# bdaiinstitute/vlfm

Measured on AMD Instinct MI355X. Metric: env-steps/s (VLM+value-map update), 640x480 RGB-D, higher is better.
Workload: dtype f16 ViT-g (f32 accumulate) + f32 Q-Former (split-f16, 22-bit); f32 confidence + f64 value maps; 1 GPU; configs[1] step x resident envs: BLIP-2 ITC + ValueMap+ObstacleMap+sort_waypoints; envs_per_gpu=256, global_envs=256, map=1000x1000 @ 20 px/m, parallelism=env-sharded x1, tuned_gemms=True, vit_gemm=hip:fc1, attention=hip

## Files before the change

### include/vlfm_amd.h

```cpp
#ifndef VLFM_AMD_H
#define VLFM_AMD_H

#include <stddef.h>
#include <stdint.h>

#ifdef __cplusplus
extern "C" {
#endif

typedef enum {
    VLFM_OK = 0,
    VLFM_ERR_INVALID = -1,
    VLFM_ERR_OUTSIDE_MAP = -2,
    VLFM_ERR_INDEX = -3,
    VLFM_ERR_HIP = -4,
    VLFM_ERR_CAPACITY = -5
} vlfm_status;

enum { VLFM_FUSE_DEFAULT = 0, VLFM_FUSE_REPLACE = 1, VLFM_FUSE_EQUAL_WEIGHTING = 2 };

const char* vlfm_last_error(void);
int vlfm_abi_version(void);

int vlfm_profile_enable(int on);
// ... 127 lines not shown
                                int out_dtype, int patch_size, void* stream);

int vlfm_itc_head_batched(const float* d_proj, int batch, int n_query, int proj_dim,
                          const float* d_text, float* d_out, void* stream);

#define VLFM_ITC_MAX_PROMPTS 8
int vlfm_itc_head_multi(const float* d_proj, int batch, int n_query, int proj_dim, const float* d_text_table, int n_text,
                        const int32_t* d_text_index, int n_prompts, float* d_out, void* stream);

int vlfm_layernorm_bias_f16(const void* d_x, const float* d_channel_bias, const void* d_gamma, const void* d_beta,
                            void* d_y, int rows, int dim, float eps, void* stream);

int vlfm_vit_attention_f16(const void* d_qkv, void* d_out, int batch, int tokens, int heads, int head_dim, float scale,
                           void* stream);

int vlfm_gemm_f16_nt(const void* d_x, const void* d_w, const void* d_bias, void* d_c, int m, int n, int k, int epilogue,
                     void* stream);

int vlfm_gemm_f16_pair_f32_nt(const void* d_x, const void* d_w_pair, const void* d_bias_f32, void* d_out, int m, int n_out, int k,
                              void* stream);

int vlfm_qformer_cross_attention_f32(const void* d_q, const void* d_kv_blocks, void* d_out, int batch, int tokens, int queries,
                                     int heads, int k_block0, int v_block0, int m_total, float scale, void* stream);

int vlfm_gemm_f16_tile_order(int m, int n, int group_m, int* out, int capacity_pairs);
int vlfm_gemm_f16_work_items(int m, int n, int grid, int* out, int capacity_pairs);

int vlfm_split_f32_to_f16_pair(const float* d_src, void* d_hi, void* d_lo, long long count, int* d_overflow, void* stream);
int vlfm_gemm_f32_nt(const float* d_x, const float* d_w, const float* d_bias, const float* d_residual, float* d_c, int m, int n,
                     int k, int activation, int precision, const void* d_w_hi, const void* d_w_lo, int* d_overflow, void* stream);


int vlfm_layernorm_rows_f32(const float* d_x, const float* d_gamma, const float* d_beta, float* d_out, int batch, int height,
                            int width, int channels, int window, float eps, void* stream);
int vlfm_window_reverse_add_f32(float* d_x, const float* d_windows, int batch, int height, int width, int channels, int window,
                                void* stream);
int vlfm_dwconv3x3_nhwc_f32(const float* d_x, const float* d_w9c, const float* d_bias, float* d_out, int batch, int height, int width,
                            int channels, void* stream);
int vlfm_window_attention_f32(const float* d_qkv, const float* d_bias_t, float* d_out, long long windows, int tokens, int heads,
                              float scale, void* stream);
int vlfm_layernorm_rows_shifted_f32(const float* d_x, const float* d_gamma, const float* d_beta, float* d_out, int batch, int height,
                                    int width, int channels, int window, float eps, int shift, int pad_zero, void* stream);
int vlfm_window_reverse_add_shifted_f32(float* d_x, const float* d_windows, int batch, int height, int width, int channels, int window,
                                        int shift, void* stream);
int vlfm_window_attention_masked_f32(const float* d_qkv, const float* d_bias_t, const float* d_mask_t, int windows_per_image, float* d_out,
                                     long long windows, int tokens, int heads, float scale, void* stream);
// ... 183 lines not shown
```

### vlfm_amd/_lib.py

```python
from __future__ import annotations

import ctypes
import os
import subprocess
from typing import Optional

_HERE = os.path.dirname(os.path.abspath(__file__))
LIB_PATH = os.path.join(_HERE, "libvlfm_amd.so")
SOURCES = ["value_map.hip", "depth_ingest.hip", "depth_holes.hip", "obstacle_map.hip", "vlm_ops.hip", "vit_attention.hip", "qformer_attention.hip", "detect_ops.hip", "object_cloud.hip", "gemm_f16.hip", "gemm_f32.hip", "conv_nhwc.hip", "sam_ops.hip", "map_render.hip", "jpeg_codec.hip", "jpeg_entropy.hip", "jpeg_decode.hip", "world_render.hip", "host.cpp"]

VLFM_OK = 0
VLFM_ERR_INVALID = -1
VLFM_ERR_OUTSIDE_MAP = -2
VLFM_ERR_INDEX = -3
VLFM_ERR_HIP = -4
VLFM_ERR_CAPACITY = -5

FUSION_TYPES = {"default": 0, "replace": 1, "equal_weighting": 2}


class VmPose(ctypes.Structure):
    _fields_ = [("inv_affine", ctypes.c_double * 6), ("row0", ctypes.c_int32), ("col0", ctypes.c_int32),
                ("env", ctypes.c_int32), ("reserved", ctypes.c_int32)]

# ... 78 lines not shown
        L.vlfm_profile_enable.argtypes = [ci]
        L.vlfm_host_wait_mode.argtypes = [ci]
        L.vlfm_profile_read.argtypes = [ctypes.c_char_p, ctypes.POINTER(cd), ctypes.POINTER(ci)]
        L.vlfm_value_map_pose_params.argtypes = [vp, vp, vp, ci, ci, ci, ci, vp, ctypes.POINTER(ci)]
        L.vlfm_cone_template_host.argtypes = [cd, cd, ci, cd, vp, ci, vp, ci, ctypes.POINTER(ci)]
        L.vlfm_tan_table_host.argtypes = [cd, ci, vp]
        L.vlfm_disc_rows_host.argtypes = [ci, vp]
        L.vlfm_cone_template_build.argtypes = [vp, vp, ci, ci, vp, vp, vp]
        L.vlfm_depth_ingest_batched.argtypes = [vp, ci, ci, ci, vp, vp, vp, ci, ci, vp, vp, vp, vp, vp]
        L.vlfm_selftest_div_exact.argtypes = [vp, ci, cd, vp, vp]
        L.vlfm_hole_scratch_bytes.argtypes = [ci, ci, ci, ci, ci]
        L.vlfm_hole_scratch_bytes.restype = ctypes.c_size_t
        L.vlfm_fill_small_holes_batched.argtypes = [vp, vp, ci, ci, ci, cd, vp, ctypes.c_size_t, ci, ci, vp, vp, vp, vp,
                                                    ci, vp, vp]
        L.vlfm_depth_scatter_holes_batched.argtypes = [vp, ci, ci, ci, vp, vp, vp, vp, ci, ci, vp, vp, vp]
        L.vlfm_fill_small_holes_rig_batched.argtypes = [vp, vp, ci, ci, ci, cd, vp, ctypes.c_size_t, ci, ci, vp, vp, vp, vp,
                                                        ci, vp, vp, ci, vp]
        L.vlfm_depth_scatter_holes_rig_batched.argtypes = [vp, ci, ci, ci, vp, vp, vp, vp, ci, ci, vp, vp, vp, vp]
        L.vlfm_layernorm_bias_f16.argtypes = [vp, vp, vp, vp, vp, ci, ci, ctypes.c_float, vp]
        L.vlfm_vit_attention_f16.argtypes = [vp, vp, ci, ci, ci, ci, ctypes.c_float, vp]
        L.vlfm_gemm_f16_nt.argtypes = [vp, vp, vp, vp, ci, ci, ci, ci, vp]
        L.vlfm_gemm_f16_pair_f32_nt.argtypes = [vp, vp, vp, vp, ci, ci, ci, vp]
        L.vlfm_qformer_cross_attention_f32.argtypes = [vp, vp, vp, ci, ci, ci, ci, ci, ci, ci, ctypes.c_float, vp]
        L.vlfm_gemm_f32_nt.argtypes = [vp, vp, vp, vp, vp, ci, ci, ci, ci, ci, vp, vp, vp, vp]
        L.vlfm_split_f32_to_f16_pair.argtypes = [vp, vp, vp, ctypes.c_longlong, vp, vp]
        L.vlfm_layernorm_rows_f32.argtypes = [vp, vp, vp, vp, ci, ci, ci, ci, ci, ctypes.c_float, vp]
        L.vlfm_window_reverse_add_f32.argtypes = [vp, vp, ci, ci, ci, ci, ci, vp]
        L.vlfm_dwconv3x3_nhwc_f32.argtypes = [vp, vp, vp, vp, ci, ci, ci, ci, vp]
        L.vlfm_window_attention_f32.argtypes = [vp, vp, vp, ctypes.c_longlong, ci, ci, ctypes.c_float, vp]
        L.vlfm_layernorm_rows_shifted_f32.argtypes = [vp, vp, vp, vp, ci, ci, ci, ci, ci, ctypes.c_float, ci, ci, vp]
        L.vlfm_window_reverse_add_shifted_f32.argtypes = [vp, vp, ci, ci, ci, ci, ci, ci, vp]
        L.vlfm_window_attention_masked_f32.argtypes = [vp, vp, vp, ci, vp, ctypes.c_longlong, ci, ci, ctypes.c_float, vp]
        L.vlfm_maxpool2x2_nhwc_f16.argtypes = [vp, vp, ci, ci, ci, ci, vp]
        L.vlfm_conv_nhwc_tile.argtypes = [ci, ci, ci, ci, ctypes.POINTER(ci), ctypes.POINTER(ci)]
        L.vlfm_conv_nhwc_f16.argtypes = [vp, vp, vp, vp, vp, ci, ci, ci, ci, ci, ci, ci, ci, ci, ci, vp]
        L.vlfm_value_map_update_fused_batched.argtypes = [vp, ci, vp, vp, vp, ci, vp, vp, ci, vp, vp, ci, ci, ci, cd, cd,
                                                          ci, ci, vp, vp, vp, vp, vp]
        L.vlfm_value_map_update_rig_batched.argtypes = [vp, ci, vp, vp, vp, ci, ci, ci, vp, vp, vp, ci, ci, ci, ci, ci, vp, vp,
                                                        vp, vp]
        L.vlfm_value_map_sort_waypoints_batched.argtypes = [vp, ci, ci, vp, ci, ci, vp, ci, vp, vp]
        L.vlfm_resample_coeffs_host.argtypes = [ci, ci, vp, vp, ci, ctypes.POINTER(ci)]
        L.vlfm_resample_coeffs_filter_host.argtypes = [ci, ci, ci, vp, vp, ci, ctypes.POINTER(ci)]
        L.vlfm_preprocess_sam_batched.argtypes = [vp, ci, ci, ci, ci, ci, vp, vp, ci, vp, vp, ci, vp, vp, ci, vp, vp, vp]
        L.vlfm_preprocess_rgb_batched.argtypes = [vp, ci, ci, ci, ci, vp, vp, ci, vp, vp, ci, vp, vp, vp, vp, ci, ci, vp]
        L.vlfm_itc_head_batched.argtypes = [vp, ci, ci, ci, vp, vp, vp]
        L.vlfm_itc_head_multi.argtypes = [vp, ci, ci, ci, vp, ci, vp, ci, vp, vp]
# ... 104 lines not shown
```

### vlfm_amd/csrc/host.cpp

```cpp
#include <cmath>
#include <cstdint>
#include <cstring>
#include <mutex>
#include <string>

#include "../../include/vlfm_amd.h"
#include "status.h"

namespace vlfm {
static thread_local std::string g_last_error;
void set_last_error(const char* msg) { g_last_error = msg ? msg : ""; }
}

extern "C" const char* vlfm_last_error(void) { return vlfm::g_last_error.c_str(); }
extern "C" int vlfm_abi_version(void) { return 16; }

namespace {

const double kPi = 3.141592653589793238462643383279502884;

inline long round_half_even(double v) { return std::lrint(v); }

float sin_deg_table(int deg) {
    static float tab[451];
    static std::once_flag once;
    std::call_once(once, [] {
        for (int i = 0; i <= 450; i++) tab[i] = (float)(std::round(std::sin(i * kPi / 180.0) * 1e7) / 1e7);
    });
    return tab[deg];
}

}

extern "C" int vlfm_value_map_pose_params(const double* h_tf, const double* h_yaw, const int32_t* h_env, int n,
                                          int map_size, int pixels_per_meter, int template_size,
                                          vlfm_vm_pose* h_out, int* bad_index) {
    if (!h_tf || !h_out || n < 0 || map_size <= 0 || template_size <= 0)
        return vlfm::fail(VLFM_ERR_INVALID, "value_map_pose_params: bad argument");
// ... 255 lines not shown
```

### vlfm_amd/csrc/qformer_attention.hip

```cpp
#include <hip/hip_runtime.h>
#include <stdint.h>

#include "../../include/vlfm_amd.h"
#include "profile.h"
#include "status.h"

namespace vlfm {

typedef float qa_f32x16 __attribute__((ext_vector_type(16)));
typedef float qa_f32x4 __attribute__((ext_vector_type(4)));
using qa_lds_ptr = __attribute__((address_space(3))) unsigned char*;
using qa_gbl_ptr = const __attribute__((address_space(1))) unsigned char*;

constexpr int QA_ROWB = 256;
constexpr int QA_MERGE_REGS = 34;
constexpr int QA_MERGE = 3 * QA_MERGE_REGS * 64 * 4;
constexpr int QA_MAX_T = 257, QA_MAX_Q = 32;

struct QaArgs {
    const float* q;
    const float* kv;
    float* out;
    int B, T, Q, heads, k_block0, v_block0, M_total;
    int rows_pad;
    float scale_log2e;
};

struct QaKernel {
    const QaArgs& a;
    unsigned char* smem;
    qa_lds_ptr lds;
    int lane, wave, col, g, voff;

    __device__ QaKernel(const QaArgs& a_, unsigned char* smem_) : a(a_), smem(smem_), lds((qa_lds_ptr)smem_) {
        lane = threadIdx.x & 63;
        wave = __builtin_amdgcn_readfirstlane(threadIdx.x >> 6);
        col = lane & 31;
        g = lane >> 5;
        voff = a.rows_pad * QA_ROWB;
    }
    __device__ inline const unsigned char* block(int block0, int b, int h) const {
        return reinterpret_cast<const unsigned char*>(a.kv + ((size_t)(block0 + h) * (size_t)a.M_total + (size_t)b * (size_t)a.T) * 64);
    }
    __device__ inline void issue_k(const unsigned char* kg, int row0, int n_ins) const {
        const int r4 = lane >> 4, p = lane & 15;
        for (int ins = 0; ins < n_ins; ins++) {
            const int row = row0 + 4 * ins + r4, src_row = min(row, a.T - 1);
            const int dst = __builtin_amdgcn_readfirstlane((row0 + 4 * ins) * QA_ROWB);
            __builtin_amdgcn_global_load_lds((qa_gbl_ptr)(kg + (size_t)src_row * QA_ROWB + ((p ^ (row & 15)) << 4)), lds + dst, 16, 0, 0);
        }
    }
    __device__ inline void issue_v(const unsigned char* vg, int row0, int n_ins) const {
        const int r4 = lane >> 4, p = lane & 15;
        for (int ins = 0; ins < n_ins; ins++) {
            const int row = row0 + 4 * ins + r4, src_row = min(row, a.T - 1);
            const int dst = __builtin_amdgcn_readfirstlane(voff + (row0 + 4 * ins) * QA_ROWB);
            __builtin_amdgcn_global_load_lds((qa_gbl_ptr)(vg + (size_t)src_row * QA_ROWB + ((p ^ (((row >> 2) & 1) << 3)) << 4)),
                                             lds + dst, 16, 0, 0);
        }
    }
    __device__ inline void issue_rows(const unsigned char* kg, const unsigned char* vg, int row0, int n_ins) const {
        issue_k(kg, row0, n_ins);
        issue_v(vg, row0, n_ins);
    }
    __device__ inline void load_q(int b, int h, float (&qn)[32]) const {
        const float* src = a.q + ((size_t)b * a.Q + min(col, a.Q - 1)) * ((size_t)a.heads * 64) + (size_t)h * 64 + 32 * g;
#pragma unroll
        for (int c = 0; c < 8; c++) {
            const qa_f32x4 v = *reinterpret_cast<const qa_f32x4*>(src + 4 * c);
            qn[4 * c] = v[0]; qn[4 * c + 1] = v[1]; qn[4 * c + 2] = v[2]; qn[4 * c + 3] = v[3];
        }
    }
};

__device__ __forceinline__ void qa_item(int w, int heads, int& b, int& h) {
    const int xcd = w & 7, idx = w >> 3;
    b = (idx / heads) * 8 + xcd;
    h = idx % heads;
}

__global__ __launch_bounds__(256) void qformer_cross_attention_kernel(QaArgs a) {
    extern __shared__ __attribute__((aligned(16))) unsigned char smem[];
    QaKernel k(a, smem);
    const int lane = k.lane, wave = k.wave, col = k.col, g = k.g;
    const int n_full = a.T >> 5, n_left = a.T & 31, left_wave = n_full & 3, left_ins = (n_left + 3) >> 2;
    const int stride = gridDim.x;
    const int moff = 2 * k.voff;
    int w = blockIdx.x, b, h;
    qa_item(w, a.heads, b, h);
// ... 132 lines not shown
                }
            }
            if (col < a.Q) {
                const float inv = 1.0f / l;
                float* orow = a.out + ((size_t)b * a.Q + col) * ((size_t)a.heads * 64) + (size_t)h * 64 + 4 * g;
#pragma unroll
                for (int q4 = 0; q4 < 4; q4++) {
                    const qa_f32x4 s0 = {o0[4 * q4] * inv, o0[4 * q4 + 1] * inv, o0[4 * q4 + 2] * inv, o0[4 * q4 + 3] * inv};
                    const qa_f32x4 s1 = {o1[4 * q4] * inv, o1[4 * q4 + 1] * inv, o1[4 * q4 + 2] * inv, o1[4 * q4 + 3] * inv};
                    *reinterpret_cast<qa_f32x4*>(orow + 8 * q4) = s0;
                    *reinterpret_cast<qa_f32x4*>(orow + 32 + 8 * q4) = s1;
                }
            }
            __builtin_amdgcn_s_waitcnt(0xC07F);
        }
        asm volatile("" ::: "memory");
        __builtin_amdgcn_s_barrier();
        asm volatile("" ::: "memory");
        if (!more) break;
        w = nw; b = nb; h = nh;
    }
}

}

using namespace vlfm;

extern "C" int vlfm_qformer_cross_attention_f32(const void* d_q, const void* d_kv_blocks, void* d_out, int batch, int tokens,
                                                int queries, int heads, int k_block0, int v_block0, int m_total, float scale,
                                                void* stream) {
    if (batch == 0) return VLFM_OK;
    if (!d_q || !d_kv_blocks || !d_out || batch < 0 || tokens < 1 || tokens > QA_MAX_T || queries < 1 || queries > QA_MAX_Q || heads < 1 ||
        k_block0 < 0 || v_block0 < 0 || (long long)batch * tokens > (long long)m_total)
        return fail(VLFM_ERR_INVALID, "qformer_cross_attention_f32: head width 64, 1-32 queries, 1-257 tokens, batch * tokens <= m_total");
    if ((((uintptr_t)d_q | (uintptr_t)d_kv_blocks | (uintptr_t)d_out) & 15) != 0)
        return fail(VLFM_ERR_INVALID, "qformer_cross_attention_f32: pointers must be 16-byte aligned");
    QaArgs a;
    a.q = (const float*)d_q; a.kv = (const float*)d_kv_blocks; a.out = (float*)d_out;
    a.B = batch; a.T = tokens; a.Q = queries; a.heads = heads; a.k_block0 = k_block0; a.v_block0 = v_block0; a.M_total = m_total;
    a.rows_pad = (tokens + 3) & ~3;
    a.scale_log2e = scale * 1.4426950408889634f;
    const size_t lds = 2 * (size_t)a.rows_pad * QA_ROWB + QA_MERGE;
    const void* fn = reinterpret_cast<const void*>(qformer_cross_attention_kernel);
    static LdsOptIn opt;
    if (!opt.ensure(fn, lds)) return fail(VLFM_ERR_HIP, "qformer_cross_attention_f32: cannot opt in to the LDS size");
    const long long items = (long long)((batch + 7) / 8) * 8 * heads;
    const int n_cu = device_cu_count() & ~7;
    const dim3 grid((unsigned)(items < n_cu ? items : n_cu)), block(256);
    VLFM_TIMED("qformer_cross_attention_kernel", stream);
    VLFM_KLAUNCH(qformer_cross_attention_kernel, grid, block, lds, stream, a);
    return check_launch("qformer_cross_attention_kernel");
}
```

### vlfm_amd/csrc/vlm_ops.hip

```cpp
#include <hip/hip_fp16.h>
#include <hip/hip_bf16.h>
#include <hip/hip_runtime.h>
#include <stdint.h>

#include <cmath>
#include <cstdlib>
#include <vector>

#include "../../include/vlfm_amd.h"
#include "profile.h"
#include "status.h"

namespace vlfm {

constexpr int PRECISION_BITS = 32 - 8 - 2;

__device__ inline unsigned char clip8(int v) {
    v >>= PRECISION_BITS;
    return (unsigned char)(v < 0 ? 0 : v > 255 ? 255 : v);
}

__global__ __launch_bounds__(256) void resample_h_kernel(const unsigned char* __restrict__ src, int H, int W, int O,
                                                         const int* __restrict__ bounds, const int* __restrict__ kk,
                                                         int ksize, unsigned char* __restrict__ dst) {
// ... 267 lines not shown
                }
            }
        }
#pragma unroll
        for (int off = 32; off > 0; off >>= 1) sq += __shfl_xor(sq, off, 64);
        const float rstd = rsqrtf(sq * inv_d + eps);
#pragma unroll
        for (int i = 0; i < NV; i++) {
            const int v = lane + 64 * i;
            if (v < nvec) {
                Half8 o;
#pragma unroll
                for (int j = 0; j < 4; j++) {
                    const float2 g2 = __half22float2(gm[i].h[j]), b2 = __half22float2(bt[i].h[j]);
                    o.h[j] = __floats2half2_rn((val(cur, i, 2 * j) - mean) * rstd * g2.x + b2.x,
                                               (val(cur, i, 2 * j + 1) - mean) * rstd * g2.y + b2.y);
                }
                reinterpret_cast<Half8*>(y + (size_t)r * D)[v] = o;
            }
        }
#pragma unroll
        for (int i = 0; i < NV; i++) { cur[i] = nxt[i]; nxt[i] = nx2[i]; }
    }
}

__global__ __launch_bounds__(512) void itc_head_kernel(const float* __restrict__ proj, int NQ, int P,
                                                       const float* __restrict__ text, float* __restrict__ out) {
    __shared__ float cos_q[64];
    const int b = blockIdx.x, lane = threadIdx.x & 63, wave = threadIdx.x >> 6, n_waves = blockDim.x >> 6;
    const float* t = text + (size_t)b * P;
    for (int q = wave; q < NQ; q += n_waves) {
        const float* p = proj + ((size_t)b * NQ + q) * P;
        float n2 = 0.0f, dt = 0.0f;
        for (int j = lane; j < P; j += 64) {
            const float v = p[j];
            n2 = fmaf(v, v, n2);
            dt = fmaf(v, t[j], dt);
        }
        for (int off = 32; off > 0; off >>= 1) {
            n2 += __shfl_down(n2, off, 64);
            dt += __shfl_down(dt, off, 64);
        }
        if (lane == 0) cos_q[q] = dt / fmaxf(sqrtf(n2), 1e-12f);
    }
    __syncthreads();
    if (wave == 0) {
// ... 235 lines not shown
}

extern "C" int vlfm_layernorm_bias_f16(const void* d_x, const float* d_channel_bias, const void* d_gamma, const void* d_beta,
                                       void* d_y, int rows, int dim, float eps, void* stream) {
    if (rows == 0) return VLFM_OK;
    if (!d_x || !d_gamma || !d_beta || !d_y || rows < 0 || dim <= 0 || dim % 8 != 0 || dim > 64 * 8 * LN_MAXV)
        return fail(VLFM_ERR_INVALID, "layernorm_bias_f16: dim must be a multiple of 8 and <= 2048");
    const int nvec = dim / 8, nv = (nvec + 63) / 64;
    int rpw = rows / 8192;
    rpw = rpw < 1 ? 1 : rpw > LN_ROWS ? LN_ROWS : rpw;
    const int waves = (rows + rpw - 1) / rpw;
    const dim3 grid((waves + 3) / 4), block(256);
    const __half* x = (const __half*)d_x; const __half* g = (const __half*)d_gamma; const __half* b = (const __half*)d_beta;
    __half* y = (__half*)d_y;
    VLFM_TIMED("layernorm_bias_f16_kernel", stream);
    switch (nv) {
        case 1: VLFM_KLAUNCH(layernorm_bias_f16_kernel<1>, grid, block, 0, (hipStream_t)stream, x, d_channel_bias, g, b, y, rows, dim, eps, rpw); break;
        case 2: VLFM_KLAUNCH(layernorm_bias_f16_kernel<2>, grid, block, 0, (hipStream_t)stream, x, d_channel_bias, g, b, y, rows, dim, eps, rpw); break;
        case 3: VLFM_KLAUNCH(layernorm_bias_f16_kernel<3>, grid, block, 0, (hipStream_t)stream, x, d_channel_bias, g, b, y, rows, dim, eps, rpw); break;
        default: VLFM_KLAUNCH(layernorm_bias_f16_kernel<4>, grid, block, 0, (hipStream_t)stream, x, d_channel_bias, g, b, y, rows, dim, eps, rpw); break;
    }
    return check_launch("layernorm_bias_f16_kernel");
}
```

### vlfm_amd/vlm/blip2itm.py

```python
from __future__ import annotations

import hashlib
import math
import os
import re
from dataclasses import dataclass
from typing import Dict, List, Optional, Sequence, Tuple

import numpy as np
import torch
import torch.nn as nn
import torch.nn.functional as F


@dataclass
class Blip2ITCConfig:
    image_size: int = 224
    patch_size: int = 14
    v_hidden: int = 1408
    v_layers: int = 39
    v_heads: int = 16
    v_mlp: int = 6144
    v_ln_eps: float = 1e-6
    q_hidden: int = 768
# ... 173 lines not shown

class _BertAttention(nn.Module):
    def __init__(self, hidden: int, kv_hidden: int, heads: int, eps: float):
        super().__init__()
        self.heads = heads
        self.query = nn.Linear(hidden, hidden)
        self.key = nn.Linear(kv_hidden, hidden)
        self.value = nn.Linear(kv_hidden, hidden)
        self.dense = nn.Linear(hidden, hidden)
        self.LayerNorm = nn.LayerNorm(hidden, eps=eps)
        self._kv_split = None
        self._qkv_fused = None

    def _project_kv_f16(self, kv16: torch.Tensor) -> Tuple[torch.Tensor, torch.Tensor]:
        if self._kv_split is None or self._kv_split[0].device != kv16.device:
            w1, w2, w3 = _exact_split3(torch.cat([self.key.weight, self.value.weight]))
            bias = torch.cat([self.key.bias, self.value.bias]).detach().float()
            self._kv_split = (w1.t(), w2.t(), w3.t(), bias)
        o = _split_gemm(kv16.reshape(-1, kv16.shape[-1]), self._kv_split[:3], self._kv_split[3])
        o = o.view(*kv16.shape[:-1], -1)
        hid = self.key.out_features
        return o[..., :hid], o[..., hid:]

    def forward(self, x: torch.Tensor, kv: Optional[torch.Tensor] = None, mask: Optional[torch.Tensor] = None,
                kv_proj: Optional[Tuple[torch.Tensor, torch.Tensor]] = None, kv_blocks=None) -> torch.Tensor:
        b, n, d = x.shape
        h = self.heads
        if kv_blocks is not None:
            from . import ops

            blocks, tokens, k_block0, v_block0 = kv_blocks
            q = _qlinear(x, self.query.weight, self.query.bias).contiguous()
            a = ops.qformer_cross_attention(q, blocks, tokens, h, k_block0, v_block0, (d // h) ** -0.5)
            return self.LayerNorm(_qlinear(a, self.dense.weight, self.dense.bias, residual=x))
        if kv_proj is not None:
            q = _qlinear(x, self.query.weight, self.query.bias).view(b, n, h, d // h).transpose(1, 2)
            k = kv_proj[0].reshape(b, -1, h, d // h).transpose(1, 2)
            v = kv_proj[1].reshape(b, -1, h, d // h).transpose(1, 2)
        elif kv is None and x.is_cuda and not self.training:
            if self._qkv_fused is None or self._qkv_fused[0].device != x.device or self._qkv_fused[0].dtype != x.dtype:
                self._qkv_fused = (torch.cat([self.query.weight, self.key.weight, self.value.weight]).detach(),
                                   torch.cat([self.query.bias, self.key.bias, self.value.bias]).detach())
            qkv = _qlinear(x, *self._qkv_fused).view(b, n, 3, h, d // h).permute(2, 0, 3, 1, 4)
            q, k, v = qkv[0], qkv[1], qkv[2]
        else:
            q = self.query(x).view(b, n, h, d // h).transpose(1, 2)
            if kv is not None and kv.dtype == torch.float16 and kv.is_cuda and self.key.weight.dtype == torch.float32:
                k, v = self._project_kv_f16(kv)
                src_len = kv.shape[1]
            else:
                src = x if kv is None else kv.to(x.dtype)
                k, v, src_len = self.key(src), self.value(src), src.shape[1]
            k = k.reshape(b, src_len, h, d // h).transpose(1, 2)
            v = v.reshape(b, src_len, h, d // h).transpose(1, 2)
        a = F.scaled_dot_product_attention(q, k, v, attn_mask=mask)
        return self.LayerNorm(_qlinear(a.transpose(1, 2).reshape(b, n, d), self.dense.weight, self.dense.bias,
                                       residual=x))


class _BertFFN(nn.Module):
    def __init__(self, hidden: int, inter: int, eps: float):
        super().__init__()
        self.up = nn.Linear(hidden, inter)
        self.down = nn.Linear(inter, hidden)
        self.LayerNorm = nn.LayerNorm(hidden, eps=eps)

# ... 17 lines not shown
    def __init__(self, cfg: Blip2ITCConfig):
        super().__init__()
        c = self.cfg = cfg
        n_patches = (c.image_size // c.patch_size) ** 2
        self.class_embedding = nn.Parameter(torch.zeros(1, 1, c.v_hidden))
        self.position_embedding = nn.Parameter(torch.zeros(1, n_patches + 1, c.v_hidden))
        self.patch_embedding = nn.Conv2d(3, c.v_hidden, c.patch_size, c.patch_size)
        self.blocks = nn.ModuleList([_VitBlock(c) for _ in range(c.v_layers)])
        self.post_layernorm = nn.LayerNorm(c.v_hidden, eps=c.v_ln_eps)
        self.query_tokens = nn.Parameter(torch.zeros(1, c.num_query_tokens, c.q_hidden))
        self.word_embeddings = nn.Embedding(c.vocab_size, c.q_hidden)
        self.position_embeddings = nn.Embedding(c.max_position_embeddings, c.q_hidden)
        self.q_layernorm = nn.LayerNorm(c.q_hidden, eps=c.q_ln_eps)
        self.q_layers = nn.ModuleList([_QFormerLayer(c, i) for i in range(c.q_layers)])
        self.vision_projection = nn.Linear(c.q_hidden, c.proj_dim)
        self.text_projection = nn.Linear(c.q_hidden, c.proj_dim)
        self.deferred_bias = True
        self._deferred_c: Optional[torch.Tensor] = None
        self.split_kv = True
        self.split_kv_min_rows = 32 * 257
        self._kv_all = None
        self.fused_cross_kv = True
        self._kv_pair = None

    def init_random(self, seed: int = 0) -> "Blip2ITCModel":
        dev = self.query_tokens.device
        g = torch.Generator(device=dev).manual_seed(seed)
        with torch.no_grad():
            for p in self.parameters():
                if p.dim() > 1:
                    p.copy_(torch.randn(p.shape, generator=g, device=dev) * 0.02)
                else:
                    p.zero_()
            for m in self.modules():
                if isinstance(m, nn.LayerNorm):
                    m.weight.fill_(1.0)
        self.weights_changed()
        return self

    def weights_changed(self) -> None:
        self._deferred_c = None
        self._kv_all = None
        self._kv_pair = None
        for layer in self.q_layers:
            layer.attention._qkv_fused = None
            if layer.crossattention is not None:
                layer.crossattention._kv_split = None

    def vision_dtype(self) -> torch.dtype:
        return self.patch_embedding.weight.dtype

    def set_precision(self, vision_dtype: torch.dtype = torch.float16) -> "Blip2ITCModel":
        for m in (self.patch_embedding, self.blocks, self.post_layernorm):
            m.to(vision_dtype)
        self.class_embedding.data = self.class_embedding.data.to(vision_dtype)
        self.position_embedding.data = self.position_embedding.data.to(vision_dtype)
        self.weights_changed()
        return self

    def load_hf_state_dict(self, sd: Dict[str, torch.Tensor]) -> None:
        own = dict(self.named_parameters())

        def put(name: str, src: str) -> None:
            with torch.no_grad():
                own[name].copy_(sd[src].to(own[name].dtype).reshape(own[name].shape))

# ... 102 lines not shown
        put("text_projection.bias", take("text_proj.bias"))
        unfed = sorted(set(own) - fed)
        if unfed:
            raise KeyError(f"{len(unfed)} parameters of the graph were not fed, e.g. {unfed[:4]}")

        def unused_ok(k: str) -> bool:
            return (k.startswith(("Qformer.cls.", "itm_head.")) or k in ("temp", "Qformer.bert.embeddings.position_ids")
                    or k.startswith(f"visual_encoder.blocks.{c.v_layers}.")
                    or k.startswith(("visual_encoder.norm.", "visual_encoder.fc_norm.", "visual_encoder.head.")))

        left = sorted(k for k in src if k not in used and not unused_ok(k))
        if left:
            raise KeyError(f"{len(left)} tensors of the file have no place in the ITC graph, e.g. {left[:4]}")
        self.weights_changed()

    def vision_tokens(self, pixel_values: torch.Tensor) -> torch.Tensor:
        c = self.cfg
        if pixel_values.dim() == 4:
            b, g = pixel_values.shape[0], c.image_size // c.patch_size
            pixel_values = pixel_values.reshape(b, 3, g, c.patch_size, g, c.patch_size).permute(0, 2, 4, 1, 3, 5) \
                .reshape(b, g * g, 3 * c.patch_size * c.patch_size)
        w = self.patch_embedding.weight
        x = F.linear(pixel_values.to(w.dtype), w.view(w.shape[0], -1), self.patch_embedding.bias)
        x = torch.cat([self.class_embedding.expand(x.shape[0], -1, -1), x], dim=1) + self.position_embedding
        if self.deferred_bias and x.is_cuda and x.dtype == torch.float16 and c.v_hidden % 8 == 0 and c.v_hidden <= 2048:
            from . import ops

            c = self._deferred_constants()
            x = x.contiguous()
            for i, blk in enumerate(self.blocks):
                x = blk.forward_deferred(x, c[2 * i], c[2 * i + 1])
            return ops.layernorm_bias(x, c[2 * len(self.blocks)], self.post_layernorm.weight, self.post_layernorm.bias,
                                      self.post_layernorm.eps)
        for blk in self.blocks:
            x = blk(x)
        return self.post_layernorm(x)

    def _deferred_constants(self) -> torch.Tensor:
        if self._deferred_c is None or self._deferred_c.device != self.post_layernorm.weight.device:
            rows, run = [], torch.zeros(self.cfg.v_hidden, dtype=torch.float32, device=self.post_layernorm.weight.device)
            for blk in self.blocks:
                rows.append(run.clone())
                run = run + blk.projection.bias.detach().float()
                rows.append(run.clone())
                run = run + blk.fc2.bias.detach().float()
            rows.append(run.clone())
            self._deferred_c = torch.stack(rows).contiguous()
        return self._deferred_c

    def query_features(self, image_tokens: torch.Tensor) -> torch.Tensor:
        split_ok = (self.split_kv and image_tokens.dtype == torch.float16 and image_tokens.is_cuda
                    and image_tokens.shape[0] * image_tokens.shape[1] >= self.split_kv_min_rows)
        enc = image_tokens if split_ok else image_tokens.to(self.q_layernorm.weight.dtype)
        h = self.q_layernorm(self.query_tokens).expand(enc.shape[0], -1, -1)
        fused = split_ok and self._fused_cross_ok(enc)
        blocks = self._project_all_kv_blocks(enc) if fused else None
        proj = self._project_all_kv(enc) if split_ok and not fused else None
        hid, at = self.cfg.q_hidden, 0
        for layer in self.q_layers:
            h = layer.attention(h)
            if layer.crossattention is not None:
                if blocks is not None:
                    h = layer.crossattention(h, kv_blocks=(blocks, enc.shape[1], at // 64, (at + hid) // 64))
                    at += 2 * hid
                elif proj is not None:
                    h = layer.crossattention(h, kv_proj=(proj[..., at:at + hid], proj[..., at + hid:at + 2 * hid]))
                    at += 2 * hid
                else:
                    h = layer.crossattention(h, kv=enc)
            h = layer.ffn_query(h)
        return h

    def _fused_cross_ok(self, tokens16: torch.Tensor) -> bool:
        from . import ops

        c = self.cfg
        return (self.fused_cross_kv and KV_SPLIT_PIECES == 2 and not torch.is_grad_enabled()
                and self.q_layernorm.weight.dtype == torch.float32
                and c.q_hidden % c.q_heads == 0 and c.q_hidden // c.q_heads == ops.QFORMER_ATTENTION_HEAD
                and c.num_query_tokens <= ops.QFORMER_ATTENTION_MAX_QUERIES
                and 1 <= tokens16.shape[1] <= ops.QFORMER_ATTENTION_MAX_TOKENS and c.v_hidden % 64 == 0
                and tokens16.shape[0] * tokens16.shape[1] * c.v_hidden * 2 < (1 << 32))

    def _kv_all_pieces(self, device):
        if self._kv_all is None or self._kv_all[0].device != device:
            cross = [l.crossattention for l in self.q_layers if l.crossattention is not None]
            w = torch.cat([torch.cat([c.key.weight, c.value.weight]) for c in cross])
            bias = torch.cat([torch.cat([c.key.bias, c.value.bias]) for c in cross]).detach().float()
            w1, w2, w3 = _exact_split3(w)
            self._kv_all = (w1.t(), w2.t(), w3.t(), bias)
            self._kv_pair = None
        return self._kv_all

    def _project_all_kv_blocks(self, tokens16: torch.Tensor) -> torch.Tensor:
        from . import ops

        w1t, w2t, _, bias = self._kv_all_pieces(tokens16.device)
        if self._kv_pair is None:
            self._kv_pair = (ops.interleave_pair_weights(w1t.t(), w2t.t()), bias.contiguous())
        return ops.linear_pair_f32(tokens16.reshape(-1, tokens16.shape[-1]), *self._kv_pair)

    def _project_all_kv(self, tokens16: torch.Tensor) -> torch.Tensor:
        pieces = self._kv_all_pieces(tokens16.device)
        o = _split_gemm(tokens16.reshape(-1, tokens16.shape[-1]), pieces[:3], pieces[3])
        return o.view(*tokens16.shape[:-1], -1)
# ... 303 lines not shown
```

### vlfm_amd/vlm/ops.py

```python
from __future__ import annotations

import ctypes
from typing import Dict, Optional, Tuple

import numpy as np
import torch

from .. import _lib

CLIP_MEAN = (0.48145466, 0.4578275, 0.40821073)
CLIP_STD = (0.26862954, 0.26130258, 0.27577711)
_DTYPE_CODE = {torch.float32: 0, torch.float16: 1, torch.bfloat16: 2}
_coeff_cache: Dict[Tuple[str, int, int], Tuple[torch.Tensor, torch.Tensor, int]] = {}


def _stream() -> int:
    return torch._C._cuda_getCurrentRawStream(torch._C._cuda_getDevice())


def resample_coeffs(in_size: int, out_size: int, bilinear: bool = False) -> Tuple[np.ndarray, np.ndarray, int]:
    bounds = np.zeros((out_size, 2), np.int32)
    cap = out_size * (2 * int(np.ceil(2.0 * max(1.0, in_size / out_size))) + 1)
    kk = np.zeros(cap, np.int32)
    ks = ctypes.c_int(0)
# ... 258 lines not shown
    return torch.stack([w1.reshape(n // 64, 64, k), w2.reshape(n // 64, 64, k)], dim=1).reshape(2 * n, k).contiguous()


def linear_pair_f32(x: torch.Tensor, w_pair: torch.Tensor, bias: Optional[torch.Tensor] = None,
                    out: Optional[torch.Tensor] = None) -> torch.Tensor:
    assert x.is_cuda and x.dtype == torch.float16 and x.is_contiguous() and x.dim() == 2
    assert w_pair.dtype == torch.float16 and w_pair.is_contiguous() and w_pair.shape[1] == x.shape[1] and w_pair.shape[0] % 128 == 0
    M, K = x.shape
    N = w_pair.shape[0] // 2
    assert bias is None or (bias.dtype == torch.float32 and bias.is_contiguous() and bias.numel() == N)
    if out is None:
        out = torch.empty((N // 64, M, 64), dtype=torch.float32, device=x.device)
    else:
        assert out.dtype == torch.float32 and out.is_contiguous() and out.shape == (N // 64, M, 64) and out.device == x.device
    _lib.check(_lib.lib().vlfm_gemm_f16_pair_f32_nt(x.data_ptr(), w_pair.data_ptr(), bias.data_ptr() if bias is not None else None,
                                                    out.data_ptr(), M, N, K, _stream()), "gemm_f16_pair_f32_nt")
    return out


QFORMER_ATTENTION_MAX_TOKENS, QFORMER_ATTENTION_MAX_QUERIES, QFORMER_ATTENTION_HEAD = 257, 32, 64


def qformer_cross_attention(q: torch.Tensor, kv_blocks: torch.Tensor, tokens: int, heads: int, k_block0: int, v_block0: int,
                            scale: float, out: Optional[torch.Tensor] = None) -> torch.Tensor:
    assert q.is_cuda and q.dtype == torch.float32 and q.is_contiguous() and q.dim() == 3 and q.shape[2] == heads * 64
    assert kv_blocks.dtype == torch.float32 and kv_blocks.is_contiguous() and kv_blocks.dim() == 3 and kv_blocks.shape[2] == 64
    assert kv_blocks.device == q.device and max(k_block0, v_block0) + heads <= kv_blocks.shape[0] and min(k_block0, v_block0) >= 0
    B, Q, _ = q.shape
    if out is None:
        out = torch.empty_like(q)
    else:
        assert out.dtype == torch.float32 and out.is_contiguous() and out.shape[1:] == q.shape[1:] and out.shape[0] >= B
    _lib.check(_lib.lib().vlfm_qformer_cross_attention_f32(q.data_ptr(), kv_blocks.data_ptr(), out.data_ptr(), B, tokens, Q, heads,
                                                           k_block0, v_block0, kv_blocks.shape[1], float(scale), _stream()),
               "qformer_cross_attention_f32")
    return out


VIT_ATTENTION_TOKENS, VIT_ATTENTION_HEADS = 257, (88,)


def vit_attention(qkv: torch.Tensor, batch: int, tokens: int, heads: int, head_dim: int, scale: float) -> torch.Tensor:
    assert qkv.is_cuda and qkv.dtype == torch.float16 and qkv.is_contiguous()
    assert qkv.numel() == batch * tokens * 3 * heads * head_dim
    out = torch.empty((batch * tokens, heads * head_dim), dtype=torch.float16, device=qkv.device)
    _lib.check(_lib.lib().vlfm_vit_attention_f16(qkv.data_ptr(), out.data_ptr(), batch, tokens, heads, head_dim,
                                                 float(scale), _stream()), "vit_attention_f16")
    return out


_ACT32 = {None: 0, "none": 0, "relu": 1, "gelu": 2}
GEMM_F32_PRECISION = {"exact": 0, "split": 1}
_overflow_flags: Dict[tuple, torch.Tensor] = {}
_split_cache: Dict[int, tuple] = {}


def gemm_f32_overflow_flag(device, owner: str = "") -> torch.Tensor:
    d = torch.device(device)
# ... 114 lines not shown
```

Before: 1743 env-steps/s.

## Fold Q-Former layer-0 query prefix, add native self-attention and token-assembly kernels

The first Q-Former layer's self-attention and cross-attention query projection depend only on learned query tokens, so they are precomputed once and cached. A stride-0 Q path in the cross-attention kernel lets every image share the one cached query. A fused HIP kernel now handles Q-Former self-attention for the remaining layers, and a second kernel merges the ViT cls-token concat with the position-embedding add. Together these cut per-step GEMMs, launches and temporary tensors. The cost is cached state that must be invalidated when weights change.

```diff
diff --git a/include/vlfm_amd.h b/include/vlfm_amd.h
--- a/include/vlfm_amd.h
+++ b/include/vlfm_amd.h
@@ -173,6 +173,14 @@
 
 int vlfm_qformer_cross_attention_f32(const void* d_q, const void* d_kv_blocks, void* d_out, int batch, int tokens, int queries,
                                      int heads, int k_block0, int v_block0, int m_total, float scale, void* stream);
+int vlfm_qformer_cross_attention_strided_f32(const void* d_q, long long q_image_stride, const void* d_kv_blocks, void* d_out, int batch,
+                                             int tokens, int queries, int heads, int k_block0, int v_block0, int m_total, float scale,
+                                             void* stream);
+
+int vlfm_qformer_self_attention_f32(const void* d_qkv, void* d_out, int batch, int queries, int heads, float scale, void* stream);
+
+int vlfm_vit_assemble_tokens_f16(const void* d_patch, const void* d_cls, const void* d_pos, void* d_out, int batch, int patches,
+                                 int dim, void* stream);
 
 int vlfm_gemm_f16_tile_order(int m, int n, int group_m, int* out, int capacity_pairs);
 int vlfm_gemm_f16_work_items(int m, int n, int grid, int* out, int capacity_pairs);
diff --git a/vlfm_amd/_lib.py b/vlfm_amd/_lib.py
--- a/vlfm_amd/_lib.py
+++ b/vlfm_amd/_lib.py
@@ -124,6 +124,10 @@
         L.vlfm_gemm_f16_nt.argtypes = [vp, vp, vp, vp, ci, ci, ci, ci, vp]
         L.vlfm_gemm_f16_pair_f32_nt.argtypes = [vp, vp, vp, vp, ci, ci, ci, vp]
         L.vlfm_qformer_cross_attention_f32.argtypes = [vp, vp, vp, ci, ci, ci, ci, ci, ci, ci, ctypes.c_float, vp]
+        L.vlfm_qformer_cross_attention_strided_f32.argtypes = [vp, ctypes.c_longlong, vp, vp, ci, ci, ci, ci, ci, ci, ci,
+                                                               ctypes.c_float, vp]
+        L.vlfm_qformer_self_attention_f32.argtypes = [vp, vp, ci, ci, ci, ctypes.c_float, vp]
+        L.vlfm_vit_assemble_tokens_f16.argtypes = [vp, vp, vp, vp, ci, ci, ci, vp]
         L.vlfm_gemm_f32_nt.argtypes = [vp, vp, vp, vp, vp, ci, ci, ci, ci, ci, vp, vp, vp, vp]
         L.vlfm_split_f32_to_f16_pair.argtypes = [vp, vp, vp, ctypes.c_longlong, vp, vp]
         L.vlfm_layernorm_rows_f32.argtypes = [vp, vp, vp, vp, ci, ci, ci, ci, ci, ctypes.c_float, vp]
diff --git a/vlfm_amd/csrc/host.cpp b/vlfm_amd/csrc/host.cpp
--- a/vlfm_amd/csrc/host.cpp
+++ b/vlfm_amd/csrc/host.cpp
@@ -13,7 +13,7 @@
 }
 
 extern "C" const char* vlfm_last_error(void) { return vlfm::g_last_error.c_str(); }
-extern "C" int vlfm_abi_version(void) { return 16; }
+extern "C" int vlfm_abi_version(void) { return 17; }
 
 namespace {
 
diff --git a/vlfm_amd/csrc/qformer_attention.hip b/vlfm_amd/csrc/qformer_attention.hip
--- a/vlfm_amd/csrc/qformer_attention.hip
+++ b/vlfm_amd/csrc/qformer_attention.hip
@@ -23,6 +23,7 @@
     float* out;
     int B, T, Q, heads, k_block0, v_block0, M_total;
     int rows_pad;
+    long long q_stride;
     float scale_log2e;
 };
 
@@ -64,7 +65,7 @@
         issue_v(vg, row0, n_ins);
     }
     __device__ inline void load_q(int b, int h, float (&qn)[32]) const {
-        const float* src = a.q + ((size_t)b * a.Q + min(col, a.Q - 1)) * ((size_t)a.heads * 64) + (size_t)h * 64 + 32 * g;
+        const float* src = a.q + (size_t)b * (size_t)a.q_stride + (size_t)min(col, a.Q - 1) * ((size_t)a.heads * 64) + (size_t)h * 64 + 32 * g;
 #pragma unroll
         for (int c = 0; c < 8; c++) {
             const qa_f32x4 v = *reinterpret_cast<const qa_f32x4*>(src + 4 * c);
@@ -243,23 +244,99 @@
     }
 }
 
+constexpr int QS_MAX_Q = 32;
+constexpr int QS_ROW = 68, QS_PROW = 33;
+
+__global__ __launch_bounds__(256) void qformer_self_attention_kernel(const float* __restrict__ qkv, float* __restrict__ out, int NQ,
+                                                                     int heads, float scale_log2e) {
+    __shared__ __attribute__((aligned(16))) float ks[QS_MAX_Q * QS_ROW];
+    __shared__ __attribute__((aligned(16))) float vs[QS_MAX_Q * QS_ROW];
+    __shared__ float ps[QS_MAX_Q * QS_PROW];
+    const int t = threadIdx.x, b = blockIdx.x / heads, h = blockIdx.x % heads;
+    const size_t hidden = (size_t)heads * 64, ld = 3 * hidden;
+    const float* base = qkv + (size_t)b * NQ * ld + (size_t)h * 64;
+    for (int r = t >> 4; r < NQ; r += 16) {
+        const int c = (t & 15) * 4;
+        *reinterpret_cast<qa_f32x4*>(ks + r * QS_ROW + c) = *reinterpret_cast<const qa_f32x4*>(base + r * ld + hidden + c);
+        *reinterpret_cast<qa_f32x4*>(vs + r * QS_ROW + c) = *reinterpret_cast<const qa_f32x4*>(base + r * ld + 2 * hidden + c);
+    }
+    const int i = t >> 3, part = t & 7;
+    qa_f32x4 q[16];
+    {
+        const float* qrow = base + (size_t)min(i, NQ - 1) * ld;
+#pragma unroll
+        for (int c = 0; c < 16; c++) q[c] = *reinterpret_cast<const qa_f32x4*>(qrow + 4 * c);
+    }
+    __syncthreads();
+    float s[4], m = -INFINITY;
+#pragma unroll
+    for (int jj = 0; jj < 4; jj++) {
+        const int j = part + 8 * jj;
+        s[jj] = -INFINITY;
+        if (j < NQ) {
+            qa_f32x4 acc = {0.f, 0.f, 0.f, 0.f};
+#pragma unroll
+            for (int c = 0; c < 16; c++) {
+                const qa_f32x4 k4 = *reinterpret_cast<const qa_f32x4*>(ks + j * QS_ROW + 4 * c);
+#pragma unroll
+                for (int e = 0; e < 4; e++) acc[e] = fmaf(q[c][e], k4[e], acc[e]);
+            }
+            s[jj] = (acc[0] + acc[1]) + (acc[2] + acc[3]);
+        }
+        m = fmaxf(m, s[jj]);
+    }
+#pragma unroll
+    for (int off = 1; off < 8; off <<= 1) m = fmaxf(m, __shfl_xor(m, off, 64));
+    float l = 0.f;
+#pragma unroll
+    for (int jj = 0; jj < 4; jj++) {
+        const int j = part + 8 * jj;
+        if (j < NQ) {
+            const float p = __builtin_amdgcn_exp2f((s[jj] - m) * scale_log2e);
+            l += p;
+            ps[i * QS_PROW + j] = p;
+        }
+    }
+#pragma unroll
+    for (int off = 1; off < 8; off <<= 1) l += __shfl_xor(l, off, 64);
+    __syncthreads();
+    qa_f32x4 o0 = {0.f, 0.f, 0.f, 0.f}, o1 = {0.f, 0.f, 0.f, 0.f};
+    for (int j = 0; j < NQ; j++) {
+        const float p = ps[i * QS_PROW + j];
+        const qa_f32x4 v0 = *reinterpret_cast<const qa_f32x4*>(vs + j * QS_ROW + 8 * part);
+        const qa_f32x4 v1 = *reinterpret_cast<const qa_f32x4*>(vs + j * QS_ROW + 8 * part + 4);
+#pragma unroll
+        for (int e = 0; e < 4; e++) { o0[e] = fmaf(p, v0[e], o0[e]); o1[e] = fmaf(p, v1[e], o1[e]); }
+    }
+    if (i < NQ) {
+        const float inv = 1.0f / l;
+        float* orow = out + ((size_t)b * NQ + i) * hidden + (size_t)h * 64 + 8 * part;
+        const qa_f32x4 r0 = {o0[0] * inv, o0[1] * inv, o0[2] * inv, o0[3] * inv}, r1 = {o1[0] * inv, o1[1] * inv, o1[2] * inv, o1[3] * inv};
+        *reinterpret_cast<qa_f32x4*>(orow) = r0;
+        *reinterpret_cast<qa_f32x4*>(orow + 4) = r1;
+    }
+}
+
 }
 
 using namespace vlfm;
 
-extern "C" int vlfm_qformer_cross_attention_f32(const void* d_q, const void* d_kv_blocks, void* d_out, int batch, int tokens,
-                                                int queries, int heads, int k_block0, int v_block0, int m_total, float scale,
-                                                void* stream) {
+extern "C" int vlfm_qformer_cross_attention_strided_f32(const void* d_q, long long q_image_stride, const void* d_kv_blocks, void* d_out,
+                                                        int batch, int tokens, int queries, int heads, int k_block0, int v_block0,
+                                                        int m_total, float scale, void* stream) {
     if (batch == 0) return VLFM_OK;
     if (!d_q || !d_kv_blocks || !d_out || batch < 0 || tokens < 1 || tokens > QA_MAX_T || queries < 1 || queries > QA_MAX_Q || heads < 1 ||
         k_block0 < 0 || v_block0 < 0 || (long long)batch * tokens > (long long)m_total)
         return fail(VLFM_ERR_INVALID, "qformer_cross_attention_f32: head width 64, 1-32 queries, 1-257 tokens, batch * tokens <= m_total");
+    if (q_image_stride != 0 && (q_image_stride < (long long)queries * heads * 64 || (q_image_stride & 3) != 0))
+        return fail(VLFM_ERR_INVALID, "qformer_cross_attention_f32: q stride must be 0 or a multiple of 4 floats >= queries * heads * 64");
     if ((((uintptr_t)d_q | (uintptr_t)d_kv_blocks | (uintptr_t)d_out) & 15) != 0)
         return fail(VLFM_ERR_INVALID, "qformer_cross_attention_f32: pointers must be 16-byte aligned");
     QaArgs a;
     a.q = (const float*)d_q; a.kv = (const float*)d_kv_blocks; a.out = (float*)d_out;
     a.B = batch; a.T = tokens; a.Q = queries; a.heads = heads; a.k_block0 = k_block0; a.v_block0 = v_block0; a.M_total = m_total;
     a.rows_pad = (tokens + 3) & ~3;
+    a.q_stride = q_image_stride;
     a.scale_log2e = scale * 1.4426950408889634f;
     const size_t lds = 2 * (size_t)a.rows_pad * QA_ROWB + QA_MERGE;
     const void* fn = reinterpret_cast<const void*>(qformer_cross_attention_kernel);
@@ -272,3 +349,25 @@
     VLFM_KLAUNCH(qformer_cross_attention_kernel, grid, block, lds, stream, a);
     return check_launch("qformer_cross_attention_kernel");
 }
+
+extern "C" int vlfm_qformer_cross_attention_f32(const void* d_q, const void* d_kv_blocks, void* d_out, int batch, int tokens,
+                                                int queries, int heads, int k_block0, int v_block0, int m_total, float scale,
+                                                void* stream) {
+    return vlfm_qformer_cross_attention_strided_f32(d_q, (long long)queries * heads * 64, d_kv_blocks, d_out, batch, tokens, queries,
+                                                    heads, k_block0, v_block0, m_total, scale, stream);
+}
+
+extern "C" int vlfm_qformer_self_attention_f32(const void* d_qkv, void* d_out, int batch, int queries, int heads, float scale,
+                                               void* stream) {
+    if (batch == 0) return VLFM_OK;
+    if (!d_qkv || !d_out || batch < 0 || queries < 1 || queries > QS_MAX_Q || heads < 1 || heads > 1024 ||
+        (long long)batch * heads > 0x7fffffffLL)
+        return fail(VLFM_ERR_INVALID, "qformer_self_attention_f32: head width 64, 1-32 queries, batch * heads < 2^31");
+    if ((((uintptr_t)d_qkv | (uintptr_t)d_out) & 15) != 0)
+        return fail(VLFM_ERR_INVALID, "qformer_self_attention_f32: pointers must be 16-byte aligned");
+    const dim3 grid((unsigned)(batch * heads)), block(256);
+    VLFM_TIMED("qformer_self_attention_kernel", stream);
+    VLFM_KLAUNCH(qformer_self_attention_kernel, grid, block, 0, stream, (const float*)d_qkv, (float*)d_out, queries, heads,
+                 scale * 1.4426950408889634f);
+    return check_launch("qformer_self_attention_kernel");
+}
diff --git a/vlfm_amd/csrc/vlm_ops.hip b/vlfm_amd/csrc/vlm_ops.hip
--- a/vlfm_amd/csrc/vlm_ops.hip
+++ b/vlfm_amd/csrc/vlm_ops.hip
@@ -313,6 +313,26 @@
 #pragma unroll
         for (int i = 0; i < NV; i++) { cur[i] = nxt[i]; nxt[i] = nx2[i]; }
     }
+}
+
+__global__ __launch_bounds__(256) void vit_assemble_tokens_f16_kernel(const Half8* __restrict__ patch, const Half8* __restrict__ cls,
+                                                                      const Half8* __restrict__ pos, Half8* __restrict__ out, int P,
+                                                                      int nvec, long long total) {
+    const long long idx = (long long)blockIdx.x * 256 + threadIdx.x;
+    if (idx >= total) return;
+    const int v = (int)(idx % nvec);
+    const long long row = idx / nvec;
+    const int t = (int)(row % (P + 1));
+    const long long b = row / (P + 1);
+    const Half8 x = t == 0 ? cls[v] : patch[(b * P + (t - 1)) * nvec + v];
+    const Half8 e = pos[(long long)t * nvec + v];
+    Half8 o;
+#pragma unroll
+    for (int j = 0; j < 4; j++) {
+        const float2 xf = __half22float2(x.h[j]), ef = __half22float2(e.h[j]);
+        o.h[j] = __floats2half2_rn(xf.x + ef.x, xf.y + ef.y);
+    }
+    out[idx] = o;
 }
 
 __global__ __launch_bounds__(512) void itc_head_kernel(const float* __restrict__ proj, int NQ, int P,
@@ -594,3 +614,19 @@
     }
     return check_launch("layernorm_bias_f16_kernel");
 }
+
+extern "C" int vlfm_vit_assemble_tokens_f16(const void* d_patch, const void* d_cls, const void* d_pos, void* d_out, int batch,
+                                            int patches, int dim, void* stream) {
+    if (batch == 0) return VLFM_OK;
+    if (!d_patch || !d_cls || !d_pos || !d_out || batch < 0 || patches < 1 || dim <= 0 || dim % 8 != 0)
+        return fail(VLFM_ERR_INVALID, "vit_assemble_tokens_f16: dim must be a multiple of 8, patches >= 1");
+    if ((((uintptr_t)d_patch | (uintptr_t)d_cls | (uintptr_t)d_pos | (uintptr_t)d_out) & 15) != 0)
+        return fail(VLFM_ERR_INVALID, "vit_assemble_tokens_f16: pointers must be 16-byte aligned");
+    const int nvec = dim / 8;
+    const long long total = (long long)batch * (patches + 1) * nvec, blocks = (total + 255) / 256;
+    if (blocks > 0x7fffffffLL) return fail(VLFM_ERR_INVALID, "vit_assemble_tokens_f16: more than 2^31 workgroups");
+    VLFM_TIMED("vit_assemble_tokens_f16_kernel", stream);
+    VLFM_KLAUNCH(vit_assemble_tokens_f16_kernel, dim3((unsigned)blocks), dim3(256), 0, (hipStream_t)stream, (const Half8*)d_patch,
+                 (const Half8*)d_cls, (const Half8*)d_pos, (Half8*)d_out, patches, nvec, total);
+    return check_launch("vit_assemble_tokens_f16_kernel");
+}
diff --git a/vlfm_amd/vlm/blip2itm.py b/vlfm_amd/vlm/blip2itm.py
--- a/vlfm_amd/vlm/blip2itm.py
+++ b/vlfm_amd/vlm/blip2itm.py
@@ -219,16 +219,29 @@
         hid = self.key.out_features
         return o[..., :hid], o[..., hid:]
 
+    def native_self_ok(self, x: torch.Tensor) -> bool:
+        from . import ops
+
+        n, d = x.shape[-2], x.shape[-1]
+        return (x.is_cuda and x.dtype == torch.float32 and self.query.weight.dtype == torch.float32
+                and not torch.is_grad_enabled() and d % self.heads == 0 and d // self.heads == ops.QFORMER_ATTENTION_HEAD
+                and 1 <= n <= ops.QFORMER_ATTENTION_MAX_QUERIES)
+
     def forward(self, x: torch.Tensor, kv: Optional[torch.Tensor] = None, mask: Optional[torch.Tensor] = None,
-                kv_proj: Optional[Tuple[torch.Tensor, torch.Tensor]] = None, kv_blocks=None) -> torch.Tensor:
+                kv_proj: Optional[Tuple[torch.Tensor, torch.Tensor]] = None, kv_blocks=None,
+                q_shared: Optional[torch.Tensor] = None) -> torch.Tensor:
         b, n, d = x.shape
         h = self.heads
         if kv_blocks is not None:
             from . import ops
 
             blocks, tokens, k_block0, v_block0 = kv_blocks
-            q = _qlinear(x, self.query.weight, self.query.bias).contiguous()
-            a = ops.qformer_cross_attention(q, blocks, tokens, h, k_block0, v_block0, (d // h) ** -0.5)
+            if q_shared is not None:
+                a = ops.qformer_cross_attention(q_shared, blocks, tokens, h, k_block0, v_block0, (d // h) ** -0.5, batch=b)
+            else:
+                q = _qlinear(x, self.query.weight, self.query.bias)
+                a = ops.qformer_cross_attention(q if q.is_contiguous() else q.contiguous(), blocks, tokens, h, k_block0, v_block0,
+                                                (d // h) ** -0.5)
             return self.LayerNorm(_qlinear(a, self.dense.weight, self.dense.bias, residual=x))
         if kv_proj is not None:
             q = _qlinear(x, self.query.weight, self.query.bias).view(b, n, h, d // h).transpose(1, 2)
@@ -238,7 +251,13 @@
             if self._qkv_fused is None or self._qkv_fused[0].device != x.device or self._qkv_fused[0].dtype != x.dtype:
                 self._qkv_fused = (torch.cat([self.query.weight, self.key.weight, self.value.weight]).detach(),
                                    torch.cat([self.query.bias, self.key.bias, self.value.bias]).detach())
-            qkv = _qlinear(x, *self._qkv_fused).view(b, n, 3, h, d // h).permute(2, 0, 3, 1, 4)
+            qkv = _qlinear(x, *self._qkv_fused)
+            if mask is None and self.native_self_ok(x) and qkv.is_contiguous():
+                from . import ops
+
+                a = ops.qformer_self_attention(qkv.view(b * n, 3 * d), b, n, h, (d // h) ** -0.5)
+                return self.LayerNorm(_qlinear(a.view(b, n, d), self.dense.weight, self.dense.bias, residual=x))
+            qkv = qkv.view(b, n, 3, h, d // h).permute(2, 0, 3, 1, 4)
             q, k, v = qkv[0], qkv[1], qkv[2]
         else:
             q = self.query(x).view(b, n, h, d // h).transpose(1, 2)
@@ -302,6 +321,9 @@
         self._kv_all = None
         self.fused_cross_kv = True
         self._kv_pair = None
+        self.fold_query_prefix = True
+        self._prefix = None
+        self._prefix_residual = {}
 
     def init_random(self, seed: int = 0) -> "Blip2ITCModel":
         dev = self.query_tokens.device
@@ -322,6 +344,8 @@
         self._deferred_c = None
         self._kv_all = None
         self._kv_pair = None
+        self._prefix = None
+        self._prefix_residual = {}
         for layer in self.q_layers:
             layer.attention._qkv_fused = None
             if layer.crossattention is not None:
@@ -470,12 +494,18 @@
                 .reshape(b, g * g, 3 * c.patch_size * c.patch_size)
         w = self.patch_embedding.weight
         x = F.linear(pixel_values.to(w.dtype), w.view(w.shape[0], -1), self.patch_embedding.bias)
-        x = torch.cat([self.class_embedding.expand(x.shape[0], -1, -1), x], dim=1) + self.position_embedding
+        if (x.is_cuda and x.dtype == torch.float16 and c.v_hidden % 8 == 0 and not torch.is_grad_enabled() and x.is_contiguous()
+                and self.class_embedding.dtype == self.position_embedding.dtype == torch.float16):
+            from . import ops
+
+            x = ops.vit_assemble_tokens(x.view(-1, c.v_hidden), self.class_embedding.view(-1),
+                                        self.position_embedding.view(-1, c.v_hidden), x.shape[0])
+        else:
+            x = (torch.cat([self.class_embedding.expand(x.shape[0], -1, -1), x], dim=1) + self.position_embedding).contiguous()
         if self.deferred_bias and x.is_cuda and x.dtype == torch.float16 and c.v_hidden % 8 == 0 and c.v_hidden <= 2048:
             from . import ops
 
             c = self._deferred_constants()
-            x = x.contiguous()
             for i, blk in enumerate(self.blocks):
                 x = blk.forward_deferred(x, c[2 * i], c[2 * i + 1])
             return ops.layernorm_bias(x, c[2 * len(self.blocks)], self.post_layernorm.weight, self.post_layernorm.bias,
@@ -505,7 +535,15 @@
         blocks = self._project_all_kv_blocks(enc) if fused else None
         proj = self._project_all_kv(enc) if split_ok and not fused else None
         hid, at = self.cfg.q_hidden, 0
-        for layer in self.q_layers:
+        fold = fused and self._fold_prefix_ok(enc.shape[0])
+        for i, layer in enumerate(self.q_layers):
+            if i == 0 and fold:
+                _, q0 = self._query_prefix(enc.device)
+                h = layer.crossattention(self._prefix_rows(enc.shape[0], enc.device), q_shared=q0,
+                                         kv_blocks=(blocks, enc.shape[1], at // 64, (at + hid) // 64))
+                at += 2 * hid
+                h = layer.ffn_query(h)
+                continue
             h = layer.attention(h)
             if layer.crossattention is not None:
                 if blocks is not None:
@@ -529,6 +567,32 @@
                 and c.num_query_tokens <= ops.QFORMER_ATTENTION_MAX_QUERIES
                 and 1 <= tokens16.shape[1] <= ops.QFORMER_ATTENTION_MAX_TOKENS and c.v_hidden % 64 == 0
                 and tokens16.shape[0] * tokens16.shape[1] * c.v_hidden * 2 < (1 << 32))
+
+    def _fold_prefix_ok(self, batch: int) -> bool:
+        c, layer = self.cfg, self.q_layers[0]
+        if not (self.fold_query_prefix and layer.crossattention is not None and not torch.is_grad_enabled()):
+            return False
+        return (batch * c.num_query_tokens >= QFORMER_SPLIT_MIN_ROWS >= 64 and c.q_hidden % 32 == 0
+                and layer.attention.native_self_ok(self.query_tokens.detach()))
+
+    def _query_prefix(self, device) -> Tuple[torch.Tensor, torch.Tensor]:
+        if self._prefix is None or self._prefix[0].device != device:
+            n = self.cfg.num_query_tokens
+            copies = (QFORMER_SPLIT_MIN_ROWS + n - 1) // n
+            layer = self.q_layers[0]
+            with torch.no_grad():
+                s = layer.attention(self.q_layernorm(self.query_tokens).expand(copies, -1, -1))
+                q = _qlinear(s, layer.crossattention.query.weight, layer.crossattention.query.bias)
+                self._prefix = (s[0].clone(), q[0].clone())
+            self._prefix_residual = {}
+        return self._prefix
+
+    def _prefix_rows(self, batch: int, device) -> torch.Tensor:
+        s0, _ = self._query_prefix(device)
+        rows = self._prefix_residual.get(batch)
+        if rows is None or rows.device != s0.device:
+            rows = self._prefix_residual[batch] = s0.expand(batch, -1, -1).contiguous()
+        return rows
 
     def _kv_all_pieces(self, device):
         if self._kv_all is None or self._kv_all[0].device != device:
diff --git a/vlfm_amd/vlm/ops.py b/vlfm_amd/vlm/ops.py
--- a/vlfm_amd/vlm/ops.py
+++ b/vlfm_amd/vlm/ops.py
@@ -304,18 +304,44 @@
 
 
 def qformer_cross_attention(q: torch.Tensor, kv_blocks: torch.Tensor, tokens: int, heads: int, k_block0: int, v_block0: int,
-                            scale: float, out: Optional[torch.Tensor] = None) -> torch.Tensor:
-    assert q.is_cuda and q.dtype == torch.float32 and q.is_contiguous() and q.dim() == 3 and q.shape[2] == heads * 64
+                            scale: float, out: Optional[torch.Tensor] = None, batch: Optional[int] = None) -> torch.Tensor:
+    assert q.is_cuda and q.dtype == torch.float32 and q.is_contiguous() and q.shape[-1] == heads * 64
     assert kv_blocks.dtype == torch.float32 and kv_blocks.is_contiguous() and kv_blocks.dim() == 3 and kv_blocks.shape[2] == 64
     assert kv_blocks.device == q.device and max(k_block0, v_block0) + heads <= kv_blocks.shape[0] and min(k_block0, v_block0) >= 0
-    B, Q, _ = q.shape
+    if q.dim() == 2:
+        assert batch is not None and batch >= 0
+        B, Q, stride = int(batch), q.shape[0], 0
+    else:
+        assert q.dim() == 3 and (batch is None or batch == q.shape[0])
+        B, Q, stride = q.shape[0], q.shape[1], q.shape[1] * q.shape[2]
     if out is None:
-        out = torch.empty_like(q)
-    else:
-        assert out.dtype == torch.float32 and out.is_contiguous() and out.shape[1:] == q.shape[1:] and out.shape[0] >= B
-    _lib.check(_lib.lib().vlfm_qformer_cross_attention_f32(q.data_ptr(), kv_blocks.data_ptr(), out.data_ptr(), B, tokens, Q, heads,
-                                                           k_block0, v_block0, kv_blocks.shape[1], float(scale), _stream()),
-               "qformer_cross_attention_f32")
+        out = torch.empty((B, Q, heads * 64), dtype=torch.float32, device=q.device)
+    else:
+        assert out.dtype == torch.float32 and out.is_contiguous() and out.shape[1:] == (Q, heads * 64) and out.shape[0] >= B
+    _lib.check(_lib.lib().vlfm_qformer_cross_attention_strided_f32(q.data_ptr(), stride, kv_blocks.data_ptr(), out.data_ptr(), B,
+                                                                   tokens, Q, heads, k_block0, v_block0, kv_blocks.shape[1],
+                                                                   float(scale), _stream()), "qformer_cross_attention_f32")
+    return out
+
+
+def qformer_self_attention(qkv: torch.Tensor, batch: int, queries: int, heads: int, scale: float) -> torch.Tensor:
+    assert qkv.is_cuda and qkv.dtype == torch.float32 and qkv.is_contiguous()
+    assert qkv.numel() == batch * queries * 3 * heads * 64
+    out = torch.empty((batch * queries, heads * 64), dtype=torch.float32, device=qkv.device)
+    _lib.check(_lib.lib().vlfm_qformer_self_attention_f32(qkv.data_ptr(), out.data_ptr(), batch, queries, heads, float(scale),
+                                                          _stream()), "qformer_self_attention_f32")
+    return out
+
+
+def vit_assemble_tokens(patch: torch.Tensor, cls: torch.Tensor, pos: torch.Tensor, batch: int) -> torch.Tensor:
+    for t in (patch, cls, pos):
+        assert t.is_cuda and t.dtype == torch.float16 and t.is_contiguous()
+    D = patch.shape[-1]
+    P = pos.numel() // D - 1
+    assert cls.numel() == D and pos.numel() == (P + 1) * D and patch.numel() == batch * P * D
+    out = torch.empty((batch, P + 1, D), dtype=torch.float16, device=patch.device)
+    _lib.check(_lib.lib().vlfm_vit_assemble_tokens_f16(patch.data_ptr(), cls.data_ptr(), pos.data_ptr(), out.data_ptr(), batch, P, D,
+                                                       _stream()), "vit_assemble_tokens_f16")
     return out
 
 
```

Result: no change. 1745 env-steps/s, median of 4 (+0.1%).
